# Tetramputechture/nclone

Measured on AMD Instinct MI355X. Metric: env-steps/sec (whole node) at N parallel envs, higher is better.
Workload: dtype f64

## Files before the change

nclone_amd/build_native.py:

```python
import os
import subprocess
import sys

HERE = os.path.dirname(os.path.abspath(__file__))
CSRC = os.path.join(HERE, "csrc")
OUT = os.path.join(HERE, "libnpp_amd.so")
SOURCES = ["npp_kernels.hip", "npp_render.hip", "npp_stack.hip", "npp_pool.hip", "npp_augment.hip", "npp_reach_kernel.hip", "npp_graph.hip", "npp_archive.hip", "npp_cells.hip", "npp_route.hip", "npp_episode.hip", "npp_pathmask.hip", "npp_reward.hip", "npp_waypoint.hip", "npp_demo.hip", "npp_seed.hip", "npp_goal.hip", "npp_sweep.hip", "npp_capi.cpp", "npp_level.cpp", "npp_reach.cpp",
           "npp_graph.cpp", "npp_host.cpp"]
HEADERS = ["npp_internal.hpp", "npp_level.hpp", "npp_tilequery.hpp", "npp_zoo.hpp", "npp_reach.hpp", "npp_reach_build.hpp", "npp_reach_features.hpp",
           "npp_host.hpp", "npp_zoo_layout.hpp", "npp_pool.hpp", "npp_augment.hpp", "npp_graph.hpp", "npp_minimal.hpp", "npp_archive.hpp", "npp_cells.hpp", "npp_route.hpp", "npp_episode.hpp", "npp_pathmask.hpp", "npp_reward.hpp", "npp_waypoint.hpp", "npp_demo.hpp", "npp_seed.hpp", "npp_goal.hpp", "npp_sweep.hpp", "npp_state.hpp",
           "npp_reach_tables.inc", os.path.join("..", "..", "include", "npp_amd.h")]


def needs_build():
    if not os.path.isfile(OUT):
        return True
    t = os.path.getmtime(OUT)
    for f in SOURCES + HEADERS:
        if os.path.getmtime(os.path.join(CSRC, f)) > t:
            return True
    return False


def build(force=False, verbose=False, out=None, extra_flags=()):
    if out is None and not force and not needs_build():
        return OUT
    hipcc = os.environ.get("HIPCC", "/opt/rocm/bin/hipcc")
    objdir = os.path.join(HERE, "_obj") if out is None else out + "_obj"
    out = OUT if out is None else out
    os.makedirs(objdir, exist_ok=True)
    flags = ["--offload-arch=gfx950", "-O3", "-std=c++17", "-fPIC", "-ffp-contract=off", "-fno-fast-math", "-Wall",
             "-Wno-unused-function", "-Wno-unused-value", "-Wno-unused-result", "-I", os.path.join(HERE, "..", "include")]
    flags += list(extra_flags)
    if verbose:
        flags.insert(0, "-Rpass-analysis=kernel-resource-usage")
    NOLICM = ["-mllvm", "-disable-machine-licm"]
    jobs = [("npp_kernels.hip", ["-DNPP_TU=%d" % k] + NOLICM, "npp_kernels_tu%d.o" % k) for k in range(4)]
    jobs += [("npp_render.hip", [], "npp_render.o"), ("npp_stack.hip", [], "npp_stack.o"), ("npp_pool.hip", [], "npp_pool.o"), ("npp_augment.hip", [], "npp_augment.o"), ("npp_capi.cpp", [], "npp_capi.o"), ("npp_level.cpp", [], "npp_level.o"),
             ("npp_reach_kernel.hip", [], "npp_reach_kernel.o"), ("npp_reach.cpp", [], "npp_reach.o"), ("npp_host.cpp", [], "npp_host.o"),
             ("npp_graph.hip", [], "npp_graph_kernel.o"), ("npp_graph.cpp", [], "npp_graph.o"), ("npp_archive.hip", [], "npp_archive.o"),
             ("npp_cells.hip", [], "npp_cells.o"), ("npp_route.hip", [], "npp_route.o"), ("npp_episode.hip", [], "npp_episode.o"), ("npp_pathmask.hip", [], "npp_pathmask.o"), ("npp_reward.hip", [], "npp_reward.o"), ("npp_waypoint.hip", [], "npp_waypoint.o"), ("npp_demo.hip", [], "npp_demo.o"),
             ("npp_seed.hip", [], "npp_seed.o"), ("npp_goal.hip", [], "npp_goal.o"), ("npp_sweep.hip", [], "npp_sweep.o")]
    procs = []
# ... 35 lines not shown
```

nclone_amd/csrc/npp_capi.cpp:

```cpp
#include <hip/hip_runtime_api.h>

#include <algorithm>
#include <cmath>
#include <cstdio>
#include <cstdlib>
#include <cstring>
#include <string>
#include <vector>

#include "../../include/npp_amd.h"
#include "npp_archive.hpp"
#include "npp_augment.hpp"
#include "npp_cells.hpp"
#include "npp_demo.hpp"
#include "npp_episode.hpp"
#include "npp_goal.hpp"
#include "npp_graph.hpp"
#include "npp_host.hpp"
#include "npp_internal.hpp"
#include "npp_level.hpp"
#include "npp_reach_build.hpp"
#include "npp_reward.hpp"
#include "npp_waypoint.hpp"
#include "npp_seed.hpp"
// ... 1715 lines not shown
        H.off_mov_meta = append(L.mov_meta.data(), 4 * L.mov_meta.size(), 4);
        H.off_mov_x0 = append(L.mov_x0.data(), 8 * L.mov_x0.size(), 8);
        H.off_mov_y0 = append(L.mov_y0.data(), 8 * L.mov_y0.size(), 8);
        H.off_edges = append(L.edges.data(), 4 * L.edges.size(), 8);
        H.off_door_tab = append(L.door_tab.data(), 4 * L.door_tab.size(), 4);
        H.off_ent_rank = append(L.ent_rank.data(), 2 * L.ent_rank.size(), 4);
        H.off_mov_rank = append(L.mov_rank.data(), 2 * L.mov_rank.size(), 4);
        H.off_ent_perm = append(L.ent_perm.data(), 2 * L.ent_perm.size(), 4);
        H.off_ent_ident = append(L.ent_ident.data(), 2 * L.ent_ident.size(), 4);
        H.off_keep_words = append(L.ent_keep_words.data(), 4 * L.ent_keep_words.size(), 4);
        H.off_draw_recs = append(L.draw_recs.data(), 4 * L.draw_recs.size(), 16);
        H.n_mov = (uint32_t)L.mov_meta.size();
        H.n_zdoor = (uint32_t)(L.door_tab.size() / 2);
        H.n_created = (uint32_t)L.n_created;
        H.n_balls = (uint32_t)L.n_balls;
        H.ball_first = 0;
        for (size_t m = 0; m < L.mov_meta.size(); m++)
            if ((L.mov_meta[m] & 7u) == MK_BALL) { H.ball_first = (uint32_t)m; break; }
        H.db_count = L.db_count;
        for (int k = 0; k < 5; k++) H.locked_slots[k] = L.locked_slots[k];
        next.zoo_doors = std::max(next.zoo_doors, (int)H.n_zdoor);
        next.zoo_movers = std::max(next.zoo_movers, (int)H.n_mov);
        H.n_seg = (uint32_t)L.segs.size();
        H.n_ent = (uint32_t)L.ent_x.size();
        H.n_words = (uint32_t)L.ent_init_words.size();
        H.n_think = (uint32_t)L.n_thinkable;
        H.obs_switch = L.obs_switch;
        H.obs_door = L.obs_door;
        H.spawn_x = L.spawn_x; H.spawn_y = L.spawn_y;
        if (L.obs_switch >= 0) {
            H.sw_x = L.ent_x[L.obs_switch]; H.sw_y = L.ent_y[L.obs_switch];
            H.door_x = L.ent_x[L.obs_door]; H.door_y = L.ent_y[L.obs_door];
        }
        next.n_words_max = std::max(next.n_words_max, (int)H.n_words);
        H.fits_lds = 1;
        next.hot_max = std::max(next.hot_max, hot_bytes);
    }
    zoo_block_plan(lv, next.zoo_doors, next.zoo_movers);
    for (int i = 0; i < n_levels; i++)
        if ((int)hdrs[i].n_zdoor > next.zoo_doors || (int)hdrs[i].n_mov > next.zoo_movers)
            return fail(h, NPP_ERR_STATE, "npp_load_levels: zoo block plan does not cover level " + std::to_string(i));
    next.zoo_words = zoo_words_for(next.zoo_doors, next.zoo_movers);
    {
        const Plan p = make_plan(next, h->n, std::vector<int32_t>((size_t)h->n, 0), h->lanes_per_env, h->waves_per_block, false, nullptr);
        if (lds_bytes(p.lds_hot_cap, next.n_words_max, (64 / p.g) * p.wpb, p.zoo_active ? next.zoo_words : 0) > LDS_BUDGET)
            return fail(h, NPP_ERR_INVALID, "npp_load_levels: entity tables exceed LDS");
    }
    const size_t N = (size_t)h->n;
    HIP_TRY(h, next.zoo.alloc((size_t)next.zoo_words * N));
    HIP_TRY(h, next.blob.alloc(host.size(), 16));
    HIP_TRY(h, next.hdr.alloc(n_levels));
    HIP_TRY(h, next.ent.alloc((size_t)next.n_words_max * N));
    HIP_TRY(h, hipStreamSynchronize(h->stream));
    HIP_TRY(h, hipMemset(h->env.count.get(), 0, h->env.count.bytes()));
    HIP_TRY(h, hipMemset(next.zoo.get(), 0, next.zoo.bytes()));
    HIP_TRY(h, hipMemcpy(next.blob.get(), host.data(), host.size(), hipMemcpyHostToDevice));
    HIP_TRY(h, hipMemcpy(next.hdr.get(), hdrs.data(), next.hdr.bytes(), hipMemcpyHostToDevice));
    HIP_TRY(h, hipMemset(next.ent.get(), 0, next.ent.bytes()));
    h->ls = std::move(next);
    h->ar = Archive();
    h->cells = Cells();
    h->demo = Demo();
    h->ep = Episode();
    h->rw = Reward();
    h->snap = Snapshot();
    h->pool.on = h->pool.ever = h->pool.dirty = false;
// ... 1616 lines not shown
```

nclone_amd/csrc/npp_internal.hpp:

```cpp
#pragma once
#include <hip/hip_runtime_api.h>

#include <cstdint>

#include "npp_goal.hpp"
#include "npp_state.hpp"
#include "npp_zoo_layout.hpp"

namespace npp {

enum F64Plane { F_X = 0, F_Y, F_VX, F_VY, F_VXO, F_VYO, F_FNX, F_FNY, F_CNX, F_CNY, F_SCX, F_SCY, NF64 };

struct LevelHdr {
    uint32_t off_hot;
    uint32_t hot_bytes;
    uint32_t off_ent_x;
    uint32_t off_ent_y;
    uint32_t off_ent_meta;
    uint32_t off_init_words;
    uint32_t off_tiles;
    uint32_t off_raster;
    uint32_t off_doors;
    uint32_t n_door;
    uint32_t n_seg;
    uint32_t n_ent;
    uint32_t n_words;
    uint32_t n_think;
    int32_t obs_switch;
    int32_t obs_door;
    uint32_t fits_lds;
    uint32_t has_zoo;
    uint32_t off_ent_seq;
    uint32_t off_ent_cell;
    uint32_t off_mov_meta;
    uint32_t off_mov_x0;
    uint32_t off_mov_y0;
    uint32_t off_edges;
    uint32_t off_door_tab;
    uint32_t n_mov;
    uint32_t n_zdoor;
    uint32_t n_created;
    uint32_t n_balls;
    uint32_t ball_first;
    uint32_t off_ent_rank;
    uint32_t off_mov_rank;
    uint32_t off_ent_perm;
    uint32_t off_ent_ident;
    uint32_t off_keep_words;
    uint32_t off_draw_recs;
    double db_count;
    int32_t locked_slots[5];
    int32_t pad_;
    double spawn_x, spawn_y;
    double sw_x, sw_y, door_x, door_y;
};

constexpr uint32_t HOT_SEG_START = 0;
constexpr uint32_t HOT_ENT_START = 2208;
constexpr uint32_t HOT_BOUNDS = 4416;
constexpr uint32_t HOT_SEGS = 5520;

struct StepOut {
    float *game_state;
    int8_t *action_mask;
    float *entity_pos;
    uint8_t *flags;
    float *reward;
    uint16_t *frames;
    float *terminal_state;
    float *spatial_context;
    double *positions;
    uint16_t *work;
};

struct KernelArgs {
    double *f64;
    uint32_t *u32;
    uint32_t *ent_bits;
    float *sc_cache;
    const int32_t *env_level;
    const int32_t *trunc_limit;
    const LevelHdr *hdr;
    const unsigned char *blob;
    const uint8_t *tile_canvas;
    const uint8_t *inputs;
    const uint8_t *reset_mask;
    const uint8_t *obs_mask;
    int n;
    int n_ticks;
    int n_steps;
    int mode;
    int autoreset;
    int n_words_max;
    int lanes_per_env;
    int waves_per_block;
    uint32_t lds_hot_cap;
    int lds_level;
    double *zoo;
    int zoo_words;
    int zoo_doors;
    int zoo_movers;
    int zoo_active;
    int reset_fresh;
    int fast_reset;
    int reset_auto;
    const uint32_t *wg_order;
    uint32_t *wg_cost;
    int wg_first, wg_count;
    uint8_t *phase;
    int phase_id;
    int variant;
    StepOut out;
};

constexpr int WAVE = 64;

constexpr int EDGE_WORDS_D = 142;

constexpr int LDS_SPILL_BYTES = 208;
__host__ __device__ inline size_t lds_spill_offset(uint32_t hot_cap, int n_words_max, int envs_per_block) {
    const size_t b = (size_t)hot_cap + (size_t)n_words_max * envs_per_block * 4 + (size_t)envs_per_block * 41 * 4;
    return (b + 7) & ~(size_t)7;
}
__host__ __device__ inline size_t lds_zoo_offset(uint32_t hot_cap, int n_words_max, int envs_per_block) {
    return lds_spill_offset(hot_cap, n_words_max, envs_per_block) + (size_t)envs_per_block * LDS_SPILL_BYTES;
}
inline size_t lds_bytes(uint32_t hot_cap, int n_words_max, int envs_per_block, int zoo_words = 0) {
    size_t b = lds_zoo_offset(hot_cap, n_words_max, envs_per_block);
    if (zoo_words) b += (size_t)envs_per_block * ((size_t)zoo_words * 8 + 2 * EDGE_WORDS_D * 4);
    return b;
}

hipError_t launch_step(const KernelArgs &a, hipStream_t s);
hipError_t launch_reset(const KernelArgs &a, hipStream_t s);
hipError_t launch_render(const KernelArgs &a, uint8_t *d_out, int centered, hipStream_t s, uint32_t stride = 84 * 84, uint32_t mirror = 0);
struct StackArgs {
    int n;
    int visual_k, state_k;
    int vhead, shead;
    int repeat;
    int reset_bits, reset_all;
    const uint8_t *flags;
    const float *game_state;
    const float *terminal_state;
    uint8_t *frames;
    float *state;
    float *terminal_stack;
};
hipError_t launch_stack_push(const StackArgs &a, hipStream_t s);
struct PoolArgs {
    int n;
    const uint8_t *flags;
    int bits;
    const double *cdf;
// ... 279 lines not shown
```

nclone_amd/csrc/npp_kernels.hip:

```cpp
#include <hip/hip_runtime.h>

#include <algorithm>
#include <vector>

#include <type_traits>

#include "npp_internal.hpp"
#include "npp_level.hpp"

#pragma clang fp contract(off)

namespace npp {
namespace {

constexpr double NINJA_RADIUS = 10.0;
constexpr double GRAVITY_FALL = 0.06666666666666665;
constexpr double GRAVITY_JUMP = 0.01111111111111111;
constexpr double GROUND_ACCEL = 0.06666666666666665;
constexpr double AIR_ACCEL = 0.04444444444444444;
constexpr double DRAG_REGULAR = 0.9933221725495059;
constexpr double DRAG_SLOW = 0.8617738760127536;
constexpr double FRICTION_GROUND = 0.9459290248857720;
constexpr double FRICTION_GROUND_SLOW = 0.8617738760127536;
constexpr double FRICTION_WALL = 0.9113380468927672;
constexpr double MAX_HOR_SPEED = 3.333;
constexpr int MAX_JUMP_DURATION = 45;
constexpr double MAX_SURVIVABLE_IMPACT = 6.0;
constexpr double TWO_THIRDS = 2.0 / 3;
constexpr double LEN45 = 0x1.0f876ccdf6cd9p+5;
constexpr double DIR45 = 0x1.6a09e667f3bcdp-1;
constexpr double LEN26 = 0x1.ad5336963eefcp+4;
constexpr double DIR26L = 0x1.c9f25c5bfedd9p-1;
constexpr double DIR26S = 0x1.c9f25c5bfedd9p-2;

#define DEV __device__ __forceinline__

#ifdef NPP_STAMPS
constexpr int N_STAMP = 12;
__device__ unsigned long long g_stamps[N_STAMP * 16384];
struct Stamps { unsigned long long acc[N_STAMP]; unsigned long long t0; };
#define STAMP_ARG , Stamps &st
#define STAMP_PASS , st
#define STAMP_INIT st.t0 = __builtin_amdgcn_s_memtime()
#define STAMP(i)                                                       \
    do {                                                               \
        unsigned long long _t1 = __builtin_amdgcn_s_memtime();         \
        st.acc[i] += _t1 - st.t0;                                      \
        st.t0 = __builtin_amdgcn_s_memtime();                          \
    } while (0)
#else
#define STAMP_ARG
#define STAMP_PASS
#define STAMP_INIT do { } while (0)
#define STAMP(i) do { } while (0)
#endif

struct Nj {
    double x, y, vx, vy, vxo, vyo, fnx, fny, cnx, cny;
    int fcount, ccount, fair, scf, frame, gold, doors;
// ... 683 lines not shown
            const int applied = collide_vs_tiles<G, K, ZOO>(lv, r, n, cd, xold, yold, fnsx, fnsy, cnsx, cnsy, cr STAMP_PASS);
            n.work += applied;
            zt.xcr = cr.xcr; zt.ycr = cr.ycr; zt.clen = cr.clen;
            if (!(zoo && zt.phys_near) && applied == 0 && n.x == xb && n.y == yb) break;
        }
        STAMP(4);
        if constexpr (!ZOO) {
            asm volatile("" ::: "memory");
            const double *sp = lv.spill;
            n.vxo = sp[0]; n.vyo = sp[1]; n.fnx = sp[2]; n.fny = sp[3]; n.cnx = sp[4]; n.cny = sp[5];
            const int *ip = reinterpret_cast<const int *>(sp + 8);
            n.fair = ip[0]; n.scf = ip[1]; n.frame = ip[2]; n.gold = ip[3]; n.doors = ip[4]; n.fastord = ip[5];
        }
        post_collision<G, K, ZOO>(lv, z, r, n, cd, eb, fnsx, fnsy, cnsx, cnsy, xold, yold, zt);
        STAMP(5);
    }
    ninja_think(n, zoo ? z.blk : nullptr);
    STAMP(6);
}

DEV void write_game_state(const Nj &n, int limit, float *o ) {
    double vmag = dsqrt(sq(n.vx) + sq(n.vy));
    o[0] = (float)(pymin(vmag / (MAX_HOR_SPEED * 2), 1.0) * 2 - 1);
    bool mv = vmag > 1e-6;
    o[1] = (float)(mv ? n.vx / vmag : 0.0);
    o[2] = (float)(mv ? n.vy / vmag : 0.0);
    o[3] = (n.state <= 2) ? 1.f : -1.f;
    o[4] = (n.state == 3 || n.state == 4) ? 1.f : -1.f;
    o[5] = (n.state == 5) ? 1.f : -1.f;
    o[6] = (n.state >= 6 && n.state <= 9) ? 1.f : -1.f;
    o[7] = n.airborn ? 1.f : -1.f;
    o[8] = (float)n.hor;
    o[9] = n.jump ? 1.f : -1.f;
    o[10] = (float)(((n.jbuf > 0 ? n.jbuf : 0) / 5.0) * 2 - 1);
    o[11] = (float)(((n.fbuf > 0 ? n.fbuf : 0) / 5.0) * 2 - 1);
    o[12] = (float)(((n.wbuf > 0 ? n.wbuf : 0) / 5.0) * 2 - 1);
    o[13] = (float)((n.fcount < 1 ? n.fcount : 1) * 2 - 1);
    o[14] = -1.f;
    o[15] = (float)((n.ccount < 1 ? n.ccount : 1) * 2 - 1);
    o[16] = (float)(dsqrt(sq(n.fnx) + sq(n.fny)) * 2 - 1);
    o[17] = 0.f;
    o[18] = (float)n.fny;
    double g = n.gjump ? GRAVITY_JUMP : GRAVITY_FALL;
    o[19] = (float)((g - GRAVITY_JUMP) / (GRAVITY_FALL - GRAVITY_JUMP) * 2 - 1);
    o[20] = n.walled ? 1.f : -1.f;
    o[21] = (float)n.fnx;
    o[22] = (float)n.cnx;
    o[23] = (float)n.cny;
    double drag = n.dslow ? DRAG_SLOW : DRAG_REGULAR;
    o[24] = (float)((drag - DRAG_SLOW) / (DRAG_REGULAR - DRAG_SLOW) * 2 - 1);
    o[25] = (float)((FRICTION_GROUND - FRICTION_GROUND_SLOW) / (FRICTION_GROUND - FRICTION_GROUND_SLOW) * 2 - 1);
    o[26] = (float)pymax(-1.0, pymin(1.0, (n.vx - n.vxo) / MAX_HOR_SPEED));
    o[27] = (float)pymax(-1.0, pymin(1.0, (n.vy - n.vyo) / MAX_HOR_SPEED));
    o[28] = (float)(pymin(vmag / (MAX_HOR_SPEED * 1.5), 1.0) * 2 - 1);
    o[29] = (float)(pymin(n.fair / 60.0, 1.0) * 2 - 1);
    o[30] = (float)(pymin(n.jdur / (double)MAX_JUMP_DURATION, 1.0) * 2 - 1);
    o[31] = (float)(pymin(n.scf / 30.0, 1.0) * 2 - 1);
    double ke = 0.5 * (sq(n.vx) + sq(n.vy));
    o[32] = (float)(pymin(ke / sq(MAX_HOR_SPEED), 1.0) * 2 - 1);
    o[33] = (float)((n.y / 600.0) * 2 - 1);
    double fm = dsqrt(sq(g) + sq(!n.airborn ? GROUND_ACCEL : AIR_ACCEL));
    o[34] = (float)(pymin(fm / 0.1, 1.0) * 2 - 1);
    double pke = 0.5 * (sq(n.vxo) + sq(n.vyo));
    o[35] = (float)pymax(-1.0, pymin(1.0, (ke - pke) / pymax(ke + 0.01, 0.01)));
    o[36] = (float)(pymin(n.fcount / 5.0, 1.0) * 2 - 1);
    o[37] = -1.f;
    o[38] = (float)(atan2(n.fny, n.fnx) / 3.141592653589793);
    o[39] = n.walled ? (float)n.wn : 0.f;
    o[40] = (float)(limit <= 0 ? 1.0 : pymax(0.0, (double)(limit - n.frame) / (double)limit));
}

DEV uint32_t action_mask_bits(const Nj &n) {
    uint32_t mask = 0x3f;
    bool has_active_buffer = (-1 < n.jbuf && n.jbuf < 5) || (-1 < n.fbuf && n.fbuf < 5) || (-1 < n.wbuf && n.wbuf < 5) ||
                             (-1 < n.lbuf && n.lbuf < 4);
    if (n.airborn && n.state != 3 && n.jump != 0 && !has_active_buffer) mask &= ~(8u | 16u | 32u);
    if (n.walled) {
        bool masks_dir = !n.airborn || n.state == 5 || !(n.vy >= 0);
        if (masks_dir) { if (n.wn > 0) mask &= ~2u; else if (n.wn < 0) mask &= ~4u; }
    }
    if (!mask) mask = 1;
    return mask;
}

template <int G>
DEV void write_spatial_context(const KernelArgs &a, const LevelHdr &H, Nj &n, EntBits eb, int env, int r, bool valid) {
    if (!valid) return;
    float *out = a.out.spatial_context + (size_t)env * 112;
    float *cache = a.sc_cache + (size_t)env * 48;
    const uint8_t *tiles = a.blob + H.off_tiles;
    const int col = floor12(n.x) >> 1, row = floor12(n.y) >> 1;
    for (int k = r; k < 64; k += G) {
        int rr = row - 4 + (k >> 3), cc = col - 4 + (k & 7);
        int t = 1;
        if (rr >= 0 && rr < 23 && cc >= 0 && cc < 42) {
            t = tiles[(cc + 1) * 25 + (rr + 1)];
            t = t > 37 ? 37 : t;
        }
// ... 87 lines not shown

template <bool ZOO>
DEV void episode_reset(const KernelArgs &a, const LevelHdr &H, Lv &lv, Zoo &z, Nj &n, EntBits eb, int nw, int r, int G) {
    const bool fast = a.fast_reset && !(n.fastord & FO_FRESH_BIT);
    const int episode = next_episode(n.fastord);
    lv.spawn_x = H.spawn_x; lv.spawn_y = H.spawn_y;
    spawn_state(lv, n);
    n.fastord = episode;
    if (fast) {
        n.fastord |= FO_FAST_BIT;
        lv.perm = reinterpret_cast<const uint16_t *>(a.blob + H.off_ent_perm);
        const uint32_t *keep = reinterpret_cast<const uint32_t *>(a.blob + H.off_keep_words);
        for (int w = 0; w < nw; w++) {
            const uint32_t k = keep[w];
            eb.w[w * eb.stride] = (eb.w[w * eb.stride] & k) | (lv.init_words[w] & ~k);
        }
        if constexpr (ZOO) {
            z.ent_ord = reinterpret_cast<const uint16_t *>(a.blob + H.off_ent_rank);
            if (z.on) zoo_fast_reset_block(z, r, G);
        }
    } else {
        lv.perm = reinterpret_cast<const uint16_t *>(a.blob + H.off_ent_ident);
        for (int w = 0; w < nw; w++) eb.w[w * eb.stride] = lv.init_words[w];
        if constexpr (ZOO) {
            z.ent_ord = z.ent_seq;
            if (z.on) zoo_init_block(z, r, G, false);
        }
    }
}

template <int G, bool LDS_LEVEL, bool ZOO, bool MANY, int V>
DEV void run(const KernelArgs &a, unsigned char *smem) {
    constexpr int EPW = WAVE / G;
    const int tid = threadIdx.x;
    const int wave = tid >> 6;
    const int lane = tid & 63;
    const int r = lane & (G - 1);
    const int epb = EPW * (blockDim.x >> 6);
    const int eib = wave * EPW + lane / G;
    const int blk = a.wg_order ? (int)a.wg_order[blockIdx.x + a.wg_first] : (int)blockIdx.x + a.wg_first;
    const unsigned long long wg_t0 = a.wg_cost ? __builtin_amdgcn_s_memtime() : 0ull;
    const int env0 = blk * epb;
    const int env = env0 + eib;
    const bool in_range = env < a.n;
    const bool valid = in_range && (!a.obs_mask || a.obs_mask[env] != 0);
    if (a.obs_mask && !__syncthreads_or(valid)) return;
    const int e = in_range ? env : a.n - 1;
    const int n_valid = (a.n - env0) < epb ? (a.n - env0) : epb;

    uint32_t *ew = reinterpret_cast<uint32_t *>(smem + (LDS_LEVEL ? a.lds_hot_cap : 0u));
    uint32_t *stage = ew + (size_t)a.n_words_max * epb;
    EntBits eb;
    eb.w = ew + eib;
    eb.stride = epb;

    const int lvl = LDS_LEVEL ? __builtin_amdgcn_readfirstlane(a.env_level[e]) : a.env_level[e];
    const LevelHdr &H = a.hdr[lvl];
    Lv lv;
    const unsigned char *hot = a.blob + H.off_hot;
    if (LDS_LEVEL) {
        const uint4 *src = reinterpret_cast<const uint4 *>(hot);
        uint4 *dst = reinterpret_cast<uint4 *>(smem);
        const int nvec = (int)(H.hot_bytes >> 4);
        for (int i = tid; i < nvec; i += blockDim.x) dst[i] = src[i];
        hot = smem;
    }
    lv.seg_start = reinterpret_cast<const uint16_t *>(hot + HOT_SEG_START);
    lv.ent_start = reinterpret_cast<const uint16_t *>(hot + HOT_ENT_START);
    lv.bounds = reinterpret_cast<const uint8_t *>(hot + HOT_BOUNDS);
    lv.segs = reinterpret_cast<const uint16_t *>(hot + HOT_SEGS);
    lv.ent_x = reinterpret_cast<const double *>(a.blob + H.off_ent_x);
    lv.ent_y = reinterpret_cast<const double *>(a.blob + H.off_ent_y);
    lv.ent_meta = reinterpret_cast<const uint32_t *>(a.blob + H.off_ent_meta);
    lv.init_words = reinterpret_cast<const uint32_t *>(a.blob + H.off_init_words);
    lv.n_think = H.n_think; lv.n_words = H.n_words;
    lv.obs_switch = H.obs_switch; lv.obs_door = H.obs_door;
    lv.spawn_x = 0; lv.spawn_y = 0; lv.sw_x = 0; lv.sw_y = 0; lv.door_x = 0; lv.door_y = 0;
    if constexpr (ZOO) { lv.sw_x = H.sw_x; lv.sw_y = H.sw_y; lv.door_x = H.door_x; lv.door_y = H.door_y; }
    lv.spill = reinterpret_cast<double *>(smem + lds_spill_offset(LDS_LEVEL ? a.lds_hot_cap : 0u, a.n_words_max, epb)) +
               (size_t)eib * (LDS_SPILL_BYTES / 8);

    Zoo z;
    z.on = false; z.blk = nullptr; z.edges = nullptr; z.n_mov = 0; z.n_door = 0; z.n_balls = 0;
    if constexpr (ZOO) {
// ... 2 lines not shown
        z.edges = reinterpret_cast<uint32_t *>(smem + zoff + (size_t)epb * a.zoo_words * 8) + (size_t)eib * (2 * EDGE_WORDS_D);
        const uint32_t ovr = reinterpret_cast<const uint32_t *>(a.zoo + (size_t)e * a.zoo_words + 3)[0];
        z.on = H.has_zoo != 0 || (ovr & (ZOO_OVR_SWITCH | ZOO_OVR_DOOR)) != 0;
        z.obs_switch = H.obs_switch; z.obs_door = H.obs_door; z.vsw_cell = -1; z.vdoor_cell = -1;
        z.ent_seq = reinterpret_cast<const uint16_t *>(a.blob + H.off_ent_seq);
        z.ent_ord = z.ent_seq;
        z.mov_rank = reinterpret_cast<const uint16_t *>(a.blob + H.off_mov_rank);
        z.ent_cell = reinterpret_cast<const uint16_t *>(a.blob + H.off_ent_cell);
        z.mov_meta = reinterpret_cast<const uint32_t *>(a.blob + H.off_mov_meta);
        z.mov_x0 = reinterpret_cast<const double *>(a.blob + H.off_mov_x0);
        z.mov_y0 = reinterpret_cast<const double *>(a.blob + H.off_mov_y0);
        z.door_tab = reinterpret_cast<const uint32_t *>(a.blob + H.off_door_tab);
        z.n_mov = (int)H.n_mov; z.n_door = (int)H.n_zdoor; z.door_words = (a.zoo_doors + 1) / 2;
        z.n_balls = (int)H.n_balls; z.n_created = (int)H.n_created; z.db_count = H.db_count; z.ball_first = (int)H.ball_first;
        if (z.on) {
            const int used = ZOO_HEAD + z.door_words + ZOO_MOV_WORDS * z.n_mov;
            const double *src = a.zoo + (size_t)e * a.zoo_words;
            for (int k = r; k < used; k += G) z.blk[k] = src[k];
            const uint32_t *esrc = reinterpret_cast<const uint32_t *>(a.blob + H.off_edges);
            for (int k = r; k < 2 * EDGE_WORDS_D; k += G) z.edges[k] = esrc[k];
            if ((ovr & ZOO_OVR_SWITCH) && H.obs_switch >= 0) {
                const double *src4 = src + 4;
                lv.sw_x = src4[0]; lv.sw_y = src4[1];
                const int c = pos_cell(src4[0], src4[1]);
                if (c != (int)z.ent_cell[H.obs_switch]) z.vsw_cell = c;
            }
            if ((ovr & ZOO_OVR_DOOR) && H.obs_door >= 0) {
                lv.door_x = src[6]; lv.door_y = src[7];
                z.vdoor_cell = pos_cell(src[6], src[7]);
            }
        }
    }

#ifdef NPP_STAMPS
    Stamps st;
    for (int i = 0; i < N_STAMP; i++) st.acc[i] = 0;
#endif
    STAMP_INIT;
    Nj n;
    load_state(a, e, n);
    lv.perm = reinterpret_cast<const uint16_t *>(a.blob + ((n.fastord & FO_FAST_BIT) ? H.off_ent_perm : H.off_ent_ident));
    if constexpr (ZOO) {
        if (n.fastord & FO_FAST_BIT) z.ent_ord = reinterpret_cast<const uint16_t *>(a.blob + H.off_ent_rank);
    }
    const int nw = (int)lv.n_words;
    if (r == 0)
        for (int w = 0; w < nw; w++) eb.w[w * eb.stride] = a.ent_bits[(size_t)w * a.n + e];
    __syncthreads();

    STAMP(0);
    uint32_t flags = 0;
    int executed = 0;
    float reward = 0.f;
    bool done = false;
    const bool stepping = a.mode == 0 && a.n_ticks > 0;
    const bool writer = valid && r == 0;
    const int n_steps = MANY ? (a.n_steps > 1 ? a.n_steps : 1) : 1;
#pragma nounroll
    for (int sidx = 0; sidx < n_steps; sidx++) {
        flags = 0; executed = 0; reward = 0.f;
        n.work = 0;
        const bool had_switch = lv.obs_switch >= 0 && ent_get(eb, lv.obs_switch) == 0;
        {
            const bool gym = a.mode == 0;
            const int act = (gym && a.n_ticks > 0) ? a.inputs[(size_t)sidx * a.n + e] : 0;
            int hor = (act == 1 || act == 4) ? -1 : ((act == 2 || act == 5) ? 1 : 0);
            int jump = act >= 3 ? 1 : 0;
            bool live = valid && !(gym && (n.state == 8 || n.state == 6 || n.state == 7));
            for (int t = 0; t < a.n_ticks; t++) {
                if (!gym) {
                    const int b = a.inputs[(size_t)t * a.n + e];
// ... 9 lines not shown
                if (!__any(live)) break;
            }
        }

        STAMP(1);
        const bool sw_now = lv.obs_switch >= 0 ? ent_get(eb, lv.obs_switch) == 0 : true;
        if (n.state == 8) flags |= 1u;
        if (n.state == 6 || n.state == 7) flags |= 2u;
        if (sw_now) flags |= 4u;
        if (n.cause == 1) flags |= 16u;
        if (n.cause == 2) flags |= 32u;
        done = (flags & 3u) != 0;
        if (stepping && !done && n.frame >= a.trunc_limit[e]) { flags |= 8u; done = true; }
        if (flags & 1u) reward += 20.f;
        if (flags & 2u) reward -= 3.f;
        if (sw_now && !had_switch && lv.obs_switch >= 0) reward += 10.f;

        if (writer) {
            const size_t o = (size_t)sidx * a.n + env;
            if (a.out.flags) a.out.flags[o] = (uint8_t)flags;
            if (a.out.reward) a.out.reward[o] = reward;
            if (a.out.frames) a.out.frames[o] = (uint16_t)executed;
            if (a.out.work) a.out.work[o] = (uint16_t)(n.work > 0xffff ? 0xffff : n.work);
        }
        if (MANY && sidx + 1 < n_steps && a.autoreset && stepping && done)
            episode_reset<ZOO>(a, H, lv, z, n, eb, nw, r, G);
    }

    const bool do_reset = a.autoreset && stepping && done;
#pragma nounroll
    for (int pass = (a.out.terminal_state ? 0 : 1); pass < 2; pass++) {
        if (pass == 1 && do_reset) episode_reset<ZOO>(a, H, lv, z, n, eb, nw, r, G);
        float *gdst = pass == 0 ? a.out.terminal_state : a.out.game_state;
        if (gdst) {
            if (r == 0) write_game_state(n, a.trunc_limit[e], reinterpret_cast<float *>(stage) + eib * 41);
            __syncthreads();
            if (pass == 1 && !a.obs_mask) {
                block_store_rows(stage, reinterpret_cast<uint32_t *>(gdst + (size_t)env0 * 41), 41, n_valid);
            } else if ((pass == 1 || do_reset) && writer) {
                const uint32_t *row = stage + eib * 41;
                uint32_t *dst = reinterpret_cast<uint32_t *>(gdst + (size_t)env * 41);
                for (int k = 0; k < 41; k++) dst[k] = row[k];
            }
            __syncthreads();
        }
    }
    if (a.out.entity_pos) {
        if (r == 0) {
            float *row = reinterpret_cast<float *>(stage) + eib * 6;
            row[0] = (float)(n.x / 1056.0); row[1] = (float)(n.y / 600.0);
            row[2] = (float)((ZOO ? lv.sw_x : H.sw_x) / 1056.0); row[3] = (float)((ZOO ? lv.sw_y : H.sw_y) / 600.0);
            row[4] = (float)((ZOO ? lv.door_x : H.door_x) / 1056.0); row[5] = (float)((ZOO ? lv.door_y : H.door_y) / 600.0);
        }
        __syncthreads();
        if (!a.obs_mask) {
            block_store_rows(stage, reinterpret_cast<uint32_t *>(a.out.entity_pos + (size_t)env0 * 6), 6, n_valid);
        } else if (writer) {
            const uint32_t *row = stage + eib * 6;
            uint32_t *dst = reinterpret_cast<uint32_t *>(a.out.entity_pos + (size_t)env * 6);
            for (int k = 0; k < 6; k++) dst[k] = row[k];
        }
        __syncthreads();
    }
    if (a.out.positions && writer) {
        double *row = a.out.positions + (size_t)env * 6;
        row[0] = n.x; row[1] = n.y;
        row[2] = ZOO ? lv.sw_x : H.sw_x; row[3] = ZOO ? lv.sw_y : H.sw_y; row[4] = ZOO ? lv.door_x : H.door_x; row[5] = ZOO ? lv.door_y : H.door_y;
    }
    if (a.out.spatial_context) write_spatial_context<G>(a, H, n, eb, env, r, valid);
    if (a.out.action_mask && writer) {
        uint32_t m = action_mask_bits(n);
        int8_t *row = a.out.action_mask + (size_t)env * 6;
        for (int k = 0; k < 6; k++) row[k] = (int8_t)((m >> k) & 1u);
    }

    STAMP(7);
    if (writer) {
        store_state(a, env, n);
        for (int w = 0; w < nw; w++) a.ent_bits[(size_t)w * a.n + env] = eb.w[w * eb.stride];
    }
    if constexpr (ZOO) {
        if (valid && z.on) {
            const int used = ZOO_HEAD + z.door_words + ZOO_MOV_WORDS * z.n_mov;
            double *dst = a.zoo + (size_t)env * a.zoo_words;
            for (int k = r; k < used; k += G) dst[k] = z.blk[k];
        }
    }
    STAMP(8);
    if (a.wg_cost && lane == 0) atomicMax(&a.wg_cost[blk], (uint32_t)(__builtin_amdgcn_s_memtime() - wg_t0));
#ifdef NPP_STAMPS
    if (lane == 0) {
        unsigned gw = blockIdx.x * (blockDim.x >> 6) + wave;
        if (gw < 16384)
            for (int i = 0; i < N_STAMP; i++) g_stamps[gw * N_STAMP + i] += st.acc[i];
    }
// ... 163 lines not shown
```

nclone_amd/csrc/npp_level.cpp:

```cpp
#include "npp_level.hpp"

#include <algorithm>
#include <array>
#include <cmath>
#include <cstring>

#include "npp_state.hpp"

namespace npp {
namespace {

const uint16_t ORTHO_NEG[34] = {0x000, 0x0c3, 0x043, 0x302, 0x08c, 0x0c1, 0x0c3, 0x003, 0x000, 0x0c0, 0x0c3, 0x003,
                                0x000, 0x0c0, 0x0c3, 0x003, 0x000, 0x0c0, 0x043, 0x003, 0x000, 0x080, 0x0c3, 0x043,
                                0x080, 0x0c0, 0x0c1, 0x002, 0x000, 0x0c0, 0x0c3, 0x003, 0x002, 0x0c1};
const uint16_t ORTHO_POS[34] = {0x000, 0xc30, 0x40c, 0xc20, 0x830, 0x310, 0x000, 0xc00, 0xc30, 0x030, 0x000, 0xc00,
                                0xc30, 0x030, 0x000, 0xc00, 0xc30, 0x030, 0x000, 0x400, 0x830, 0x030, 0x400, 0xc00,
                                0xc30, 0x830, 0x000, 0xc00, 0xc20, 0x010, 0x010, 0xc20, 0xc30, 0x030};

const uint16_t GRID_EDGE[34] = {0x000, 0xcf3, 0x44f, 0xf22, 0x8bc, 0x3d1, 0x6db, 0xe67, 0xdb6, 0x9f9, 0xcf3, 0xcf3,
                                0xcf3, 0xcf3, 0x6db, 0xe67, 0xdb6, 0x9f9, 0x44f, 0x44f, 0x8bc, 0x8bc, 0xcf3, 0xcf3,
                                0xcf3, 0xcf3, 0x3d1, 0xf22, 0xf22, 0x3d1, 0xcf3, 0xcf3, 0xcf3, 0xcf3};

uint16_t pack_linear(int x1, int y1, int x2, int y2) {
    return (uint16_t)(0u | (x1 << 2) | (y1 << 4) | (x2 << 6) | (y2 << 8));
}
uint16_t pack_arc(int cx, int cy, int hor, int ver, int convex) {
    return (uint16_t)(1u | (cx << 2) | (cy << 4) | ((hor > 0) << 6) | ((ver > 0) << 7) | ((convex != 0) << 8));
}

bool tile_special(int t, uint16_t &seg) {
    switch (t) {
        case 6: seg = pack_linear(0, 2, 2, 0); return true;
        case 7: seg = pack_linear(0, 0, 2, 2); return true;
        case 8: seg = pack_linear(2, 0, 0, 2); return true;
        case 9: seg = pack_linear(2, 2, 0, 0); return true;
        case 10: seg = pack_arc(0, 0, 1, 1, 1); return true;
        case 11: seg = pack_arc(2, 0, -1, 1, 1); return true;
        case 12: seg = pack_arc(2, 2, -1, -1, 1); return true;
        case 13: seg = pack_arc(0, 2, 1, -1, 1); return true;
// ... 356 lines not shown
        });
        for (const DicRef &d : dic) L.dic_order.push_back(d.ref);
        L.ent_rank.assign(ne, 0);
        L.mov_rank.assign(movers.size(), 0);
        for (size_t k = 0; k < L.dic_order.size(); k++) {
            const uint32_t ref = L.dic_order[k];
            if (ref & 0x80000000u) L.mov_rank[ref & 0x7fffffffu] = (uint16_t)k;
            else L.ent_rank[ref] = (uint16_t)k;
        }
        if (moved_switch >= 0) L.ent_rank[slot_of[moved_switch]] = (uint16_t)next_seq;
        L.ent_perm.resize(ne);
        L.ent_ident.resize(ne);
        for (size_t s2 = 0; s2 < ne; s2++) { L.ent_perm[s2] = (uint16_t)s2; L.ent_ident[s2] = (uint16_t)s2; }
        for (int c = 0; c < N_CELLS; c++)
            std::stable_sort(L.ent_perm.begin() + L.ent_start[c], L.ent_perm.begin() + L.ent_start[c + 1], [&](uint16_t a, uint16_t b) {
                const int ka = ((L.ent_meta[a] & 15u) == EK_EXIT) ? 0x10000 : L.ent_rank[a];
                const int kb = ((L.ent_meta[b] & 15u) == EK_EXIT) ? 0x10000 : L.ent_rank[b];
                return ka < kb;
            });
        L.ent_keep_words.assign((ne + 15) / 16, 0);
        for (size_t s2 = 0; s2 < ne; s2++) {
            const uint32_t kind = L.ent_meta[s2] & 15u;
            if (kind == EK_BOOST || kind == EK_DOOR_REG) L.ent_keep_words[ent_word(s2)] |= ent_bits_at(2u, s2);
        }
    }
    {
        int k = 0;
        for (size_t i = 0; i < raw.size() && k < 5; i++)
            if (raw[i].kind == EK_LOCKED) L.locked_slots[k++] = slot_of[i];
    }
    if (last_switch_raw >= 0) {
        L.obs_switch = slot_of[last_switch_raw];
        L.obs_door = slot_of[raw[last_switch_raw].link_raw];
    }
    return true;
}

int dump_segments(const CompiledLevel &lv, int16_t *out, int max_rows) {
    int r = 0;
    for (int c = 0; c < N_CELLS; c++) {
        int cx = c / GRID_H, cy = c % GRID_H;
        for (int i = lv.seg_start[c]; i < lv.seg_start[c + 1]; i++) {
            if (r >= max_rows) return -1;
            uint16_t s = lv.segs[i];
            int16_t *o = out + 8 * r++;
            o[0] = (int16_t)cx; o[1] = (int16_t)cy; o[2] = (int16_t)(s & 1);
            if ((s & 1) == 0) {
                o[3] = (int16_t)(24 * cx + 12 * ((s >> 2) & 3)); o[4] = (int16_t)(24 * cy + 12 * ((s >> 4) & 3));
                o[5] = (int16_t)(24 * cx + 12 * ((s >> 6) & 3)); o[6] = (int16_t)(24 * cy + 12 * ((s >> 8) & 3));
                o[7] = 1;
            } else {
                o[3] = (int16_t)(24 * cx + 12 * ((s >> 2) & 3)); o[4] = (int16_t)(24 * cy + 12 * ((s >> 4) & 3));
                o[5] = (int16_t)(((s >> 6) & 1) ? 1 : -1); o[6] = (int16_t)(((s >> 7) & 1) ? 1 : -1);
                o[7] = (int16_t)((s >> 8) & 1);
            }
        }
    }
    return r;
}

}
```

nclone_amd/csrc/npp_level.hpp:

```cpp
#pragma once
#include <cstdint>
#include <string>
#include <vector>

namespace npp {

constexpr int GRID_W = 44;
constexpr int GRID_H = 25;
constexpr int N_CELLS = GRID_W * GRID_H;

enum EntKind : uint32_t { EK_NONE = 0, EK_MINE = 1, EK_GOLD = 2, EK_EXIT = 3, EK_SWITCH = 4, EK_DOOR_REG = 5, EK_LOCKED = 6,
                          EK_DOOR_TRAP = 7, EK_LAUNCH = 8, EK_ONEWAY = 9, EK_BOOST = 10 };
enum MoverKind : uint32_t { MK_DRONE = 1, MK_BOUNCE = 2, MK_THWUMP = 3, MK_BALL = 4, MK_MINI = 5, MK_SHOVE = 6 };
constexpr int EDGE_W = 89, EDGE_H = 51;
constexpr int EDGE_WORDS = (EDGE_W * EDGE_H + 31) / 32;

struct CompiledLevel {
    std::vector<uint16_t> seg_start;
    std::vector<uint16_t> segs;
    std::vector<uint8_t> cell_bounds;
    std::vector<uint16_t> ent_start;
    std::vector<double> ent_x, ent_y;
    std::vector<uint32_t> ent_meta;
    std::vector<uint16_t> ent_map_order;
    std::vector<uint32_t> ent_init_words;
    std::vector<uint8_t> tiles;
    std::vector<uint16_t> raster_order;
    std::vector<uint32_t> draw_recs;
    std::vector<double> door_segs;
    double spawn_x = 0, spawn_y = 0;
    int obs_switch = -1, obs_door = -1;
    int n_thinkable = 0;
    uint32_t unsupported_mask = 0;
    std::vector<uint16_t> ent_seq;
    std::vector<uint16_t> ent_cell;
    std::vector<uint32_t> mov_meta;
    std::vector<double> mov_x0, mov_y0;
    std::vector<uint32_t> edges;
    std::vector<uint32_t> door_tab;
    std::vector<uint32_t> dic_order;
    std::vector<uint16_t> ent_rank;
    std::vector<uint16_t> mov_rank;
    std::vector<uint16_t> ent_perm;
    std::vector<uint16_t> ent_ident;
    std::vector<uint32_t> ent_keep_words;
    int locked_slots[5] = {-1, -1, -1, -1, -1};
    int n_created = 0;
    int n_balls = 0;
    double db_count = 0;
    bool goal_variant = false;
    bool has_zoo = false;
};

bool compile_level(const double *map, int64_t n, CompiledLevel &out, std::string &err);

bool compile_level_variant(const double *map, int64_t n, const double *goal_xy, CompiledLevel &out, std::string &err);

int dump_segments(const CompiledLevel &lv, int16_t *out, int max_rows);

}
```

Before: 98.40 million.

## Precompute observation terms as constexpr tables and fuse entity_pos staging into game-state pass

Replaces the per-step double-precision divisions and sqrt in the game-state observation writer with constexpr lookup tables and precomputed constants. The static switch and door position row is computed once at level load and stored in the header. The entity_pos row gets its own LDS staging area, so its write shares the barrier with the final game-state store instead of running a separate staged loop with two extra __syncthreads. This costs more LDS per env (six extra words) and a small table lookup with index clamping.

```diff
diff --git a/nclone_amd/build_native.py b/nclone_amd/build_native.py
--- a/nclone_amd/build_native.py
+++ b/nclone_amd/build_native.py
@@ -8,7 +8,7 @@
 SOURCES = ["npp_kernels.hip", "npp_render.hip", "npp_stack.hip", "npp_pool.hip", "npp_augment.hip", "npp_reach_kernel.hip", "npp_graph.hip", "npp_archive.hip", "npp_cells.hip", "npp_route.hip", "npp_episode.hip", "npp_pathmask.hip", "npp_reward.hip", "npp_waypoint.hip", "npp_demo.hip", "npp_seed.hip", "npp_goal.hip", "npp_sweep.hip", "npp_capi.cpp", "npp_level.cpp", "npp_reach.cpp",
            "npp_graph.cpp", "npp_host.cpp"]
 HEADERS = ["npp_internal.hpp", "npp_level.hpp", "npp_tilequery.hpp", "npp_zoo.hpp", "npp_reach.hpp", "npp_reach_build.hpp", "npp_reach_features.hpp",
-           "npp_host.hpp", "npp_zoo_layout.hpp", "npp_pool.hpp", "npp_augment.hpp", "npp_graph.hpp", "npp_minimal.hpp", "npp_archive.hpp", "npp_cells.hpp", "npp_route.hpp", "npp_episode.hpp", "npp_pathmask.hpp", "npp_reward.hpp", "npp_waypoint.hpp", "npp_demo.hpp", "npp_seed.hpp", "npp_goal.hpp", "npp_sweep.hpp", "npp_state.hpp",
+           "npp_host.hpp", "npp_zoo_layout.hpp", "npp_pool.hpp", "npp_augment.hpp", "npp_graph.hpp", "npp_minimal.hpp", "npp_archive.hpp", "npp_cells.hpp", "npp_route.hpp", "npp_episode.hpp", "npp_pathmask.hpp", "npp_reward.hpp", "npp_waypoint.hpp", "npp_demo.hpp", "npp_seed.hpp", "npp_goal.hpp", "npp_sweep.hpp", "npp_state.hpp", "npp_obs_rows.hpp",
            "npp_reach_tables.inc", os.path.join("..", "..", "include", "npp_amd.h")]
 
 
diff --git a/nclone_amd/csrc/npp_capi.cpp b/nclone_amd/csrc/npp_capi.cpp
--- a/nclone_amd/csrc/npp_capi.cpp
+++ b/nclone_amd/csrc/npp_capi.cpp
@@ -1771,6 +1771,7 @@
             H.sw_x = L.ent_x[L.obs_switch]; H.sw_y = L.ent_y[L.obs_switch];
             H.door_x = L.ent_x[L.obs_door]; H.door_y = L.ent_y[L.obs_door];
         }
+        for (int k = 0; k < 4; k++) H.obs_pos[k] = L.obs_pos[k];
         next.n_words_max = std::max(next.n_words_max, (int)H.n_words);
         H.fits_lds = 1;
         next.hot_max = std::max(next.hot_max, hot_bytes);
diff --git a/nclone_amd/csrc/npp_internal.hpp b/nclone_amd/csrc/npp_internal.hpp
--- a/nclone_amd/csrc/npp_internal.hpp
+++ b/nclone_amd/csrc/npp_internal.hpp
@@ -53,6 +53,7 @@
     int32_t pad_;
     double spawn_x, spawn_y;
     double sw_x, sw_y, door_x, door_y;
+    float obs_pos[4];
 };
 
 constexpr uint32_t HOT_SEG_START = 0;
@@ -119,7 +120,7 @@
 
 constexpr int LDS_SPILL_BYTES = 208;
 __host__ __device__ inline size_t lds_spill_offset(uint32_t hot_cap, int n_words_max, int envs_per_block) {
-    const size_t b = (size_t)hot_cap + (size_t)n_words_max * envs_per_block * 4 + (size_t)envs_per_block * 41 * 4;
+    const size_t b = (size_t)hot_cap + (size_t)n_words_max * envs_per_block * 4 + (size_t)envs_per_block * (41 + 6) * 4;
     return (b + 7) & ~(size_t)7;
 }
 __host__ __device__ inline size_t lds_zoo_offset(uint32_t hot_cap, int n_words_max, int envs_per_block) {
diff --git a/nclone_amd/csrc/npp_kernels.hip b/nclone_amd/csrc/npp_kernels.hip
--- a/nclone_amd/csrc/npp_kernels.hip
+++ b/nclone_amd/csrc/npp_kernels.hip
@@ -7,6 +7,7 @@
 
 #include "npp_internal.hpp"
 #include "npp_level.hpp"
+#include "npp_obs_rows.hpp"
 
 #pragma clang fp contract(off)
 
@@ -14,17 +15,10 @@
 namespace {
 
 constexpr double NINJA_RADIUS = 10.0;
-constexpr double GRAVITY_FALL = 0.06666666666666665;
-constexpr double GRAVITY_JUMP = 0.01111111111111111;
-constexpr double GROUND_ACCEL = 0.06666666666666665;
-constexpr double AIR_ACCEL = 0.04444444444444444;
-constexpr double DRAG_REGULAR = 0.9933221725495059;
-constexpr double DRAG_SLOW = 0.8617738760127536;
 constexpr double FRICTION_GROUND = 0.9459290248857720;
 constexpr double FRICTION_GROUND_SLOW = 0.8617738760127536;
 constexpr double FRICTION_WALL = 0.9113380468927672;
 constexpr double MAX_HOR_SPEED = 3.333;
-constexpr int MAX_JUMP_DURATION = 45;
 constexpr double MAX_SURVIVABLE_IMPACT = 6.0;
 constexpr double TWO_THIRDS = 2.0 / 3;
 constexpr double LEN45 = 0x1.0f876ccdf6cd9p+5;
@@ -774,38 +768,35 @@
     o[7] = n.airborn ? 1.f : -1.f;
     o[8] = (float)n.hor;
     o[9] = n.jump ? 1.f : -1.f;
-    o[10] = (float)(((n.jbuf > 0 ? n.jbuf : 0) / 5.0) * 2 - 1);
-    o[11] = (float)(((n.fbuf > 0 ? n.fbuf : 0) / 5.0) * 2 - 1);
-    o[12] = (float)(((n.wbuf > 0 ? n.wbuf : 0) / 5.0) * 2 - 1);
+    o[10] = obs_buffer(n.jbuf);
+    o[11] = obs_buffer(n.fbuf);
+    o[12] = obs_buffer(n.wbuf);
     o[13] = (float)((n.fcount < 1 ? n.fcount : 1) * 2 - 1);
     o[14] = -1.f;
     o[15] = (float)((n.ccount < 1 ? n.ccount : 1) * 2 - 1);
     o[16] = (float)(dsqrt(sq(n.fnx) + sq(n.fny)) * 2 - 1);
     o[17] = 0.f;
     o[18] = (float)n.fny;
-    double g = n.gjump ? GRAVITY_JUMP : GRAVITY_FALL;
-    o[19] = (float)((g - GRAVITY_JUMP) / (GRAVITY_FALL - GRAVITY_JUMP) * 2 - 1);
+    o[19] = obs_gravity(n.gjump);
     o[20] = n.walled ? 1.f : -1.f;
     o[21] = (float)n.fnx;
     o[22] = (float)n.cnx;
     o[23] = (float)n.cny;
-    double drag = n.dslow ? DRAG_SLOW : DRAG_REGULAR;
-    o[24] = (float)((drag - DRAG_SLOW) / (DRAG_REGULAR - DRAG_SLOW) * 2 - 1);
+    o[24] = obs_drag(n.dslow);
     o[25] = (float)((FRICTION_GROUND - FRICTION_GROUND_SLOW) / (FRICTION_GROUND - FRICTION_GROUND_SLOW) * 2 - 1);
     o[26] = (float)pymax(-1.0, pymin(1.0, (n.vx - n.vxo) / MAX_HOR_SPEED));
     o[27] = (float)pymax(-1.0, pymin(1.0, (n.vy - n.vyo) / MAX_HOR_SPEED));
     o[28] = (float)(pymin(vmag / (MAX_HOR_SPEED * 1.5), 1.0) * 2 - 1);
-    o[29] = (float)(pymin(n.fair / 60.0, 1.0) * 2 - 1);
-    o[30] = (float)(pymin(n.jdur / (double)MAX_JUMP_DURATION, 1.0) * 2 - 1);
-    o[31] = (float)(pymin(n.scf / 30.0, 1.0) * 2 - 1);
+    o[29] = obs_fair(n.fair);
+    o[30] = obs_jdur(n.jdur);
+    o[31] = obs_scf(n.scf);
     double ke = 0.5 * (sq(n.vx) + sq(n.vy));
     o[32] = (float)(pymin(ke / sq(MAX_HOR_SPEED), 1.0) * 2 - 1);
     o[33] = (float)((n.y / 600.0) * 2 - 1);
-    double fm = dsqrt(sq(g) + sq(!n.airborn ? GROUND_ACCEL : AIR_ACCEL));
-    o[34] = (float)(pymin(fm / 0.1, 1.0) * 2 - 1);
+    o[34] = obs_force(n.gjump, n.airborn);
     double pke = 0.5 * (sq(n.vxo) + sq(n.vyo));
     o[35] = (float)pymax(-1.0, pymin(1.0, (ke - pke) / pymax(ke + 0.01, 0.01)));
-    o[36] = (float)(pymin(n.fcount / 5.0, 1.0) * 2 - 1);
+    o[36] = obs_fcount(n.fcount);
     o[37] = -1.f;
     o[38] = (float)(atan2(n.fny, n.fnx) / 3.141592653589793);
     o[39] = n.walled ? (float)n.wn : 0.f;
@@ -959,6 +950,11 @@
 template <int G, bool LDS_LEVEL, bool ZOO, bool MANY, int V>
 DEV void run(const KernelArgs &a, unsigned char *smem) {
     constexpr int EPW = WAVE / G;
+#ifdef NPP_STAMPS
+    Stamps st;
+    for (int i = 0; i < N_STAMP; i++) st.acc[i] = 0;
+#endif
+    STAMP_INIT;
     const int tid = threadIdx.x;
     const int wave = tid >> 6;
     const int lane = tid & 63;
@@ -977,6 +973,7 @@
 
     uint32_t *ew = reinterpret_cast<uint32_t *>(smem + (LDS_LEVEL ? a.lds_hot_cap : 0u));
     uint32_t *stage = ew + (size_t)a.n_words_max * epb;
+    uint32_t *stage_pos = stage + (size_t)epb * 41;
     EntBits eb;
     eb.w = ew + eib;
     eb.stride = epb;
@@ -1045,11 +1042,6 @@
         }
     }
 
-#ifdef NPP_STAMPS
-    Stamps st;
-    for (int i = 0; i < N_STAMP; i++) st.acc[i] = 0;
-#endif
-    STAMP_INIT;
     Nj n;
     load_state(a, e, n);
     lv.perm = reinterpret_cast<const uint16_t *>(a.blob + ((n.fastord & FO_FAST_BIT) ? H.off_ent_perm : H.off_ent_ident));
@@ -1125,9 +1117,22 @@
     for (int pass = (a.out.terminal_state ? 0 : 1); pass < 2; pass++) {
         if (pass == 1 && do_reset) episode_reset<ZOO>(a, H, lv, z, n, eb, nw, r, G);
         float *gdst = pass == 0 ? a.out.terminal_state : a.out.game_state;
+        float *pdst = pass == 1 ? a.out.entity_pos : nullptr;
+        if (!gdst && !pdst) continue;
+        if (r == 0) {
+            if (gdst) write_game_state(n, a.trunc_limit[e], reinterpret_cast<float *>(stage) + eib * 41);
+            if (pdst) {
+                float *row = reinterpret_cast<float *>(stage_pos) + eib * 6;
+                row[0] = obs_pos_x(n.x); row[1] = obs_pos_y(n.y);
+                if constexpr (ZOO) {
+                    row[2] = obs_pos_x(lv.sw_x); row[3] = obs_pos_y(lv.sw_y); row[4] = obs_pos_x(lv.door_x); row[5] = obs_pos_y(lv.door_y);
+                } else {
+                    row[2] = H.obs_pos[0]; row[3] = H.obs_pos[1]; row[4] = H.obs_pos[2]; row[5] = H.obs_pos[3];
+                }
+            }
+        }
+        __syncthreads();
         if (gdst) {
-            if (r == 0) write_game_state(n, a.trunc_limit[e], reinterpret_cast<float *>(stage) + eib * 41);
-            __syncthreads();
             if (pass == 1 && !a.obs_mask) {
                 block_store_rows(stage, reinterpret_cast<uint32_t *>(gdst + (size_t)env0 * 41), 41, n_valid);
             } else if ((pass == 1 || do_reset) && writer) {
@@ -1135,25 +1140,17 @@
                 uint32_t *dst = reinterpret_cast<uint32_t *>(gdst + (size_t)env * 41);
                 for (int k = 0; k < 41; k++) dst[k] = row[k];
             }
-            __syncthreads();
-        }
-    }
-    if (a.out.entity_pos) {
-        if (r == 0) {
-            float *row = reinterpret_cast<float *>(stage) + eib * 6;
-            row[0] = (float)(n.x / 1056.0); row[1] = (float)(n.y / 600.0);
-            row[2] = (float)((ZOO ? lv.sw_x : H.sw_x) / 1056.0); row[3] = (float)((ZOO ? lv.sw_y : H.sw_y) / 600.0);
-            row[4] = (float)((ZOO ? lv.door_x : H.door_x) / 1056.0); row[5] = (float)((ZOO ? lv.door_y : H.door_y) / 600.0);
-        }
-        __syncthreads();
-        if (!a.obs_mask) {
-            block_store_rows(stage, reinterpret_cast<uint32_t *>(a.out.entity_pos + (size_t)env0 * 6), 6, n_valid);
-        } else if (writer) {
-            const uint32_t *row = stage + eib * 6;
-            uint32_t *dst = reinterpret_cast<uint32_t *>(a.out.entity_pos + (size_t)env * 6);
-            for (int k = 0; k < 6; k++) dst[k] = row[k];
-        }
-        __syncthreads();
+        }
+        if (pdst) {
+            if (!a.obs_mask) {
+                block_store_rows(stage_pos, reinterpret_cast<uint32_t *>(pdst + (size_t)env0 * 6), 6, n_valid);
+            } else if (writer) {
+                const uint32_t *row = stage_pos + eib * 6;
+                uint32_t *dst = reinterpret_cast<uint32_t *>(pdst + (size_t)env * 6);
+                for (int k = 0; k < 6; k++) dst[k] = row[k];
+            }
+        }
+        if (pass == 0) __syncthreads();
     }
     if (a.out.positions && writer) {
         double *row = a.out.positions + (size_t)env * 6;
diff --git a/nclone_amd/csrc/npp_level.cpp b/nclone_amd/csrc/npp_level.cpp
--- a/nclone_amd/csrc/npp_level.cpp
+++ b/nclone_amd/csrc/npp_level.cpp
@@ -5,6 +5,7 @@
 #include <cmath>
 #include <cstring>
 
+#include "npp_obs_rows.hpp"
 #include "npp_state.hpp"
 
 namespace npp {
@@ -427,6 +428,8 @@
     if (last_switch_raw >= 0) {
         L.obs_switch = slot_of[last_switch_raw];
         L.obs_door = slot_of[raw[last_switch_raw].link_raw];
+        L.obs_pos[0] = obs_pos_x(L.ent_x[L.obs_switch]); L.obs_pos[1] = obs_pos_y(L.ent_y[L.obs_switch]);
+        L.obs_pos[2] = obs_pos_x(L.ent_x[L.obs_door]);   L.obs_pos[3] = obs_pos_y(L.ent_y[L.obs_door]);
     }
     return true;
 }
diff --git a/nclone_amd/csrc/npp_level.hpp b/nclone_amd/csrc/npp_level.hpp
--- a/nclone_amd/csrc/npp_level.hpp
+++ b/nclone_amd/csrc/npp_level.hpp
@@ -30,6 +30,7 @@
     std::vector<double> door_segs;
     double spawn_x = 0, spawn_y = 0;
     int obs_switch = -1, obs_door = -1;
+    float obs_pos[4] = {0.f, 0.f, 0.f, 0.f};
     int n_thinkable = 0;
     uint32_t unsupported_mask = 0;
     std::vector<uint16_t> ent_seq;
diff --git a/nclone_amd/csrc/npp_obs_rows.hpp b/nclone_amd/csrc/npp_obs_rows.hpp
--- /dev/null
+++ b/nclone_amd/csrc/npp_obs_rows.hpp
@@ -0,0 +1,114 @@
+#pragma once
+#include <cstdint>
+
+#include "npp_state.hpp"
+
+namespace npp {
+
+constexpr double GRAVITY_FALL = 0.06666666666666665;
+constexpr double GRAVITY_JUMP = 0.01111111111111111;
+constexpr double GROUND_ACCEL = 0.06666666666666665;
+constexpr double AIR_ACCEL = 0.04444444444444444;
+constexpr double DRAG_REGULAR = 0.9933221725495059;
+constexpr double DRAG_SLOW = 0.8617738760127536;
+constexpr int MAX_JUMP_DURATION = 45;
+
+constexpr double obs_min(double a, double b) { return b < a ? b : a; }
+
+constexpr double obs_sqrt(double x) {
+    int e = 0;
+    while (x < 4503599627370496.0) { x *= 2.0; e--; }
+    while (x >= 9007199254740992.0) { x *= 0.5; e++; }
+    unsigned __int128 m = (unsigned __int128)(uint64_t)x;
+    if (e & 1) { m <<= 1; e--; }
+    m <<= 54;
+    unsigned __int128 r = 0;
+    for (int bit = 54; bit >= 0; bit--) {
+        const unsigned __int128 t = r | ((unsigned __int128)1 << bit);
+        if (t * t <= m) r = t;
+    }
+    const bool sticky = r * r != m;
+    uint64_t q = (uint64_t)(r >> 1);
+    if ((r & 1) && (sticky || (q & 1))) q++;
+    double v = (double)q;
+    int s = (e - 54) / 2 + 1;
+    for (; s > 0; s--) v *= 2.0;
+    for (; s < 0; s++) v *= 0.5;
+    return v;
+}
+
+template <int N>
+struct ObsTable {
+    float v[N];
+};
+
+constexpr ObsTable<6> obs_make_buffer() {
+    ObsTable<6> t{};
+    for (int b = 0; b < 6; b++) t.v[b] = (float)((b / 5.0) * 2 - 1);
+    return t;
+}
+constexpr ObsTable<61> obs_make_fair() {
+    ObsTable<61> t{};
+    for (int k = 0; k <= 60; k++) t.v[k] = (float)(obs_min(k / 60.0, 1.0) * 2 - 1);
+    return t;
+}
+constexpr ObsTable<MAX_JUMP_DURATION + 1> obs_make_jdur() {
+    ObsTable<MAX_JUMP_DURATION + 1> t{};
+    for (int k = 0; k <= MAX_JUMP_DURATION; k++) t.v[k] = (float)(obs_min(k / (double)MAX_JUMP_DURATION, 1.0) * 2 - 1);
+    return t;
+}
+constexpr ObsTable<31> obs_make_scf() {
+    ObsTable<31> t{};
+    for (int k = 0; k <= 30; k++) t.v[k] = (float)(obs_min(k / 30.0, 1.0) * 2 - 1);
+    return t;
+}
+constexpr ObsTable<6> obs_make_fcount() {
+    ObsTable<6> t{};
+    for (int k = 0; k <= 5; k++) t.v[k] = (float)(obs_min(k / 5.0, 1.0) * 2 - 1);
+    return t;
+}
+
+constexpr float obs_gravity_term(double g) { return (float)((g - GRAVITY_JUMP) / (GRAVITY_FALL - GRAVITY_JUMP) * 2 - 1); }
+constexpr float obs_drag_term(double drag) { return (float)((drag - DRAG_SLOW) / (DRAG_REGULAR - DRAG_SLOW) * 2 - 1); }
+constexpr float obs_force_term(double g, double acc) { return (float)(obs_min(obs_sqrt(g * g + acc * acc) / 0.1, 1.0) * 2 - 1); }
+
+NPP_HD inline int obs_index(int v, int last) { return v < 0 ? 0 : (v > last ? last : v); }
+
+NPP_HD inline float obs_buffer(int buf) {
+    static constexpr ObsTable<6> T = obs_make_buffer();
+    return T.v[obs_index(buf, 5)];
+}
+NPP_HD inline float obs_fair(int fair) {
+    static constexpr ObsTable<61> T = obs_make_fair();
+    return T.v[obs_index(fair, 60)];
+}
+NPP_HD inline float obs_jdur(int jdur) {
+    static constexpr ObsTable<MAX_JUMP_DURATION + 1> T = obs_make_jdur();
+    return T.v[obs_index(jdur, MAX_JUMP_DURATION)];
+}
+NPP_HD inline float obs_scf(int scf) {
+    static constexpr ObsTable<31> T = obs_make_scf();
+    return T.v[obs_index(scf, 30)];
+}
+NPP_HD inline float obs_fcount(int fcount) {
+    static constexpr ObsTable<6> T = obs_make_fcount();
+    return T.v[obs_index(fcount, 5)];
+}
+NPP_HD inline float obs_gravity(bool jump_gravity) {
+    constexpr float J = obs_gravity_term(GRAVITY_JUMP), F = obs_gravity_term(GRAVITY_FALL);
+    return jump_gravity ? J : F;
+}
+NPP_HD inline float obs_drag(bool slow) {
+    constexpr float S = obs_drag_term(DRAG_SLOW), R = obs_drag_term(DRAG_REGULAR);
+    return slow ? S : R;
+}
+NPP_HD inline float obs_force(bool jump_gravity, bool airborn) {
+    constexpr float JG = obs_force_term(GRAVITY_JUMP, GROUND_ACCEL), JA = obs_force_term(GRAVITY_JUMP, AIR_ACCEL),
+                    FG = obs_force_term(GRAVITY_FALL, GROUND_ACCEL), FA = obs_force_term(GRAVITY_FALL, AIR_ACCEL);
+    return jump_gravity ? (airborn ? JA : JG) : (airborn ? FA : FG);
+}
+
+NPP_HD inline float obs_pos_x(double x) { return (float)(x / 1056.0); }
+NPP_HD inline float obs_pos_y(double y) { return (float)(y / 600.0); }
+
+}
```

Measured after the change: 99.77 million (median of 6 runs). 1.01x the previous value.
